# DmSM-1/C-OFDM

Hardware: AMD Instinct MI355X
Metric: IQ-samples/sec (tx IFFT+CP and rx FFT+equalise), 2048-subcarrier frames, 1/2/4/8 GPU (higher is better)
Workload: dtype f64

## Files before the change

### c-ofdm_amd/csrc/ofdm_capi.cpp

```cpp
#include <dlfcn.h>
#include <hip/hip_runtime.h>

#include <algorithm>
#include <climits>
#include <cmath>
#include <complex>
#include <cstdarg>
#include <cstdio>
#include <cstdlib>
#include <chrono>
#include <mutex>
#include <cstring>
#include <iterator>
#include <stdexcept>
#include <string>
#include <vector>

#include "../../include/ofdm_mi355x.h"

#if __has_include(<rccl/rccl.h>)
#include <rccl/rccl.h>
static constexpr int kRcclInt64 = ncclInt64, kRcclSum = ncclSum;
#else
static constexpr int kRcclInt64 = 4, kRcclSum = 0;
// ... 185 lines not shown
    return OFDM_OK;
}

int ofdm_host_alloc(ofdm_ctx* c, size_t bytes, void** h)
{
    if (!c || !h) return fail(OFDM_ERR_INVALID, "null argument");
    HIP_TRY(hipSetDevice(c->device));
    HIP_TRY(hipHostMalloc(h, std::max<size_t>(bytes, 1), hipHostMallocDefault));
    return OFDM_OK;
}
int ofdm_host_free(ofdm_ctx* c, void* h)
{
    if (!c) return fail(OFDM_ERR_INVALID, "null ctx");
    if (h) HIP_TRY(hipHostFree(h));
    return OFDM_OK;
}
int ofdm_stream_create(ofdm_ctx* c, void** st)
{
    if (!c || !st) return fail(OFDM_ERR_INVALID, "null argument");
    HIP_TRY(hipSetDevice(c->device));
    hipStream_t s = nullptr;
    HIP_TRY(hipStreamCreateWithFlags(&s, hipStreamNonBlocking));
    *st = s;
    return OFDM_OK;
}
int ofdm_stream_destroy(ofdm_ctx* c, void* st)
{
    if (!c) return fail(OFDM_ERR_INVALID, "null ctx");
    if (st) {
        HIP_TRY(hipStreamSynchronize((hipStream_t)st));
        rx_queue_release(c, (hipStream_t)st);
        if (c->call_valid && c->call_stream == (hipStream_t)st) c->call_valid = false;
        HIP_TRY(hipStreamDestroy((hipStream_t)st));
    }
    return OFDM_OK;
}
int ofdm_memcpy_d2d(ofdm_ctx* c, void* dst, const void* src, size_t n, void* st)
{
    if (!c) return fail(OFDM_ERR_INVALID, "null ctx");
    if (n) HIP_TRY(hipMemcpyAsync(dst, src, n, hipMemcpyDeviceToDevice, (hipStream_t)st));
    return OFDM_OK;
}
int ofdm_copy(ofdm_ctx* c, void* dst, const void* src, size_t n, void* st)
{
    if (!c) return fail(OFDM_ERR_INVALID, "null ctx");
    if (n && (!dst || !src)) return fail(OFDM_ERR_INVALID, "null argument");
    hipError_t e = ofdm::launch_copy(dst, src, n, (hipStream_t)st);
    if (e != hipSuccess) return hip_fail(e, "copy launch");
    return OFDM_OK;
}
int ofdm_event_create(ofdm_ctx* c, void** ev)
{
    if (!c || !ev) return fail(OFDM_ERR_INVALID, "null argument");
    HIP_TRY(hipSetDevice(c->device));
    hipEvent_t e = nullptr;
    HIP_TRY(hipEventCreateWithFlags(&e, hipEventDisableTiming));
    *ev = e;
    return OFDM_OK;
}
int ofdm_event_record(ofdm_ctx* c, void* ev, void* st)
{
    if (!c || !ev) return fail(OFDM_ERR_INVALID, "null argument");
    HIP_TRY(hipEventRecord((hipEvent_t)ev, (hipStream_t)st));
    return OFDM_OK;
}
int ofdm_event_synchronize(ofdm_ctx* c, void* ev)
{
    if (!c || !ev) return fail(OFDM_ERR_INVALID, "null argument");
    HIP_TRY(hipEventSynchronize((hipEvent_t)ev));
    return OFDM_OK;
}
int ofdm_event_destroy(ofdm_ctx* c, void* ev)
{
    if (!c) return fail(OFDM_ERR_INVALID, "null ctx");
    if (ev) HIP_TRY(hipEventDestroy((hipEvent_t)ev));
    return OFDM_OK;
}

static void fill_tx(const ofdm_ctx* c, ofdm::TxArgs& a, const uint8_t* bytes, size_t nframes, double* iq,
                    size_t stride, int16_t* iq16, const ofdm_channel* ch)
{
    a.tab = c->tables(false);
    a.tx_dead = c->tx_sparse ? c->d_tx_dead : nullptr;
    a.bytes = bytes;
    a.iq = reinterpret_cast<double2*>(iq);
    a.iq16 = iq16;
    a.nframes = (long)nframes;
    a.frame_stride = (long)stride;
    a.S = c->S;
    a.D = c->D;
    a.P = c->P;
    a.cp = c->cp;
    a.k = c->k;
    a.bytes_per_frame = c->geo.bytes_per_frame;
    a.pilot_ampl = (double)c->p.pilot_ampl / 1000;
    a.inv_sqrt_n = 1.0 / std::sqrt((double)c->N);
    a.mult = (double)c->p.mult;
    if (ch && ch->noise_std > 0.0) {
        a.noise_scale = ch->noise_std * M_SQRT1_2;
        a.seed = ch->seed;
        a.sample_offset = ch->sample_offset;
    }
}

int ofdm_tx_modulate(ofdm_ctx* c, const uint8_t* bytes, size_t nframes, double* iq_out, size_t frame_stride,
                     int16_t* iq16_out, const ofdm_channel* ch, void* stream)
{
    if (!c || !bytes || !iq_out) return fail(OFDM_ERR_INVALID, "null argument");
    if (frame_stride < (size_t)c->geo.message_len) return fail(OFDM_ERR_INVALID, "frame_stride < message_len");
    if (!aligned16(iq_out)) return fail(OFDM_ERR_INVALID, "iq_out must be 16-byte aligned");
    if (nframes == 0) return OFDM_OK;
    if (nframes * (size_t)c->S > 0x7fffffffu) return fail(OFDM_ERR_INVALID, "too many symbols in one call");
    ofdm::TxArgs a{};
    fill_tx(c, a, bytes, nframes, iq_out, frame_stride, iq16_out, ch);
    hipError_t e = ofdm::launch_tx(c->logn, a, (hipStream_t)stream);
    if (e != hipSuccess) return hip_fail(e, "tx_kernel launch");
    return OFDM_OK;
}

int ofdm_tx_frames(ofdm_ctx* c, const uint8_t* bytes, size_t nframes, double* frames_out, int16_t* frames16_out,
                   void* stream)
{
    if (!c || !bytes || !frames_out) return fail(OFDM_ERR_INVALID, "null argument");
    if (!aligned16(frames_out)) return fail(OFDM_ERR_INVALID, "frames_out must be 16-byte aligned");
    if (nframes == 0) return OFDM_OK;
    ofdm::TxArgs a{};
    fill_tx(c, a, bytes, nframes, frames_out, (size_t)c->geo.frame_len, frames16_out, nullptr);
    a.header = c->d_header;
    a.header_len = (int)(c->t2 + c->geo.preamble_len);
    a.msg_offset = a.header_len;
    hipError_t e = ofdm::launch_tx(c->logn, a, (hipStream_t)stream);
    if (e != hipSuccess) return hip_fail(e, "tx_kernel launch");
    return OFDM_OK;
}

}

static int rx_demod_impl(ofdm_ctx* c, const double* iq, const int16_t* iq16, size_t nframes, size_t frame_stride,
                         const double* chan, size_t chan_stride, double* constell_out, uint8_t* bytes_out,
                         const uint8_t* ref_bytes, unsigned long long* bit_errors, void* stream,
                         double* read_out = nullptr, const ofdm::SoftArgs* soft = nullptr)
{
    if (!c || (!iq && !iq16)) return fail(OFDM_ERR_INVALID, "null argument");
    if (iq16 && ((uintptr_t)iq16 & 3)) return fail(OFDM_ERR_INVALID, "iq16 must be 4-byte aligned");
    if (frame_stride < (size_t)c->geo.message_len) return fail(OFDM_ERR_INVALID, "frame_stride < message_len");
    if ((iq && !aligned16(iq)) || (chan && !aligned16(chan)) || (constell_out && !aligned16(constell_out)))
        return fail(OFDM_ERR_INVALID, "complex buffers must be 16-byte aligned");
    if ((ref_bytes == nullptr) != (bit_errors == nullptr))
        return fail(OFDM_ERR_INVALID, "ref_bytes and bit_errors go together");
    if (nframes == 0) return OFDM_OK;
    if (nframes > 0x7fffffffu) return fail(OFDM_ERR_INVALID, "too many frames in one call");
    ofdm::RxArgs a{};
    a.tab = c->tables(false);
    a.iq = iq16 ? nullptr : reinterpret_cast<const double2*>(iq);
    a.iq16 = reinterpret_cast<const short2*>(iq16);
    a.nframes = (long)nframes;
    a.frame_stride = (long)frame_stride;
    a.chan = reinterpret_cast<const double2*>(chan);
    a.chan_stride = (long)chan_stride;
    a.constell = reinterpret_cast<double2*>(constell_out);
    a.read_out = reinterpret_cast<double2*>(read_out);
    a.bytes = bytes_out;
    a.ref = ref_bytes;
    a.bit_errors = bit_errors;
    a.S = c->S;
    a.D = c->D;
// ... 1025 lines not shown
```

### c-ofdm_amd/csrc/ofdm_create.cpp

```cpp
#include <hip/hip_runtime.h>

#include <algorithm>
#include <cctype>
#include <climits>
#include <cmath>
#include <fstream>
#include <memory>
#include <string>
#include <unordered_map>
#include <vector>

#include "ofdm_ctx.hpp"
#include "ofdm_sync.hpp"
#include "ofdm_tables.hpp"

namespace tables = ofdm::tables;
using ofdm::DevBuf;
using ofdm::fail;
using ofdm::hip_fail;
using ofdm::twiddles;
using tables::ilog2_exact;

namespace {

// ... 21 lines not shown
            return fail(OFDM_ERR_PARSE, "stol failed for key '%s': %s", key.c_str(), e.what());
        }
    }
    return OFDM_OK;
}

template <class T>
int upload(DevBuf<T>& dst, const std::vector<T>& v)
{
    HIP_TRY(hipMalloc((void**)dst.put(), std::max<size_t>(1, v.size()) * sizeof(T)));
    if (!v.empty()) HIP_TRY(hipMemcpy(dst, v.data(), v.size() * sizeof(T), hipMemcpyHostToDevice));
    return OFDM_OK;
}

std::vector<double2> as_double2(const std::vector<cd>& v)
{
    std::vector<double2> o(v.size());
    for (size_t i = 0; i < v.size(); ++i) o[i] = make_double2(v[i].real(), v[i].imag());
    return o;
}

int validate(const ofdm_params* p)
{
    const long N = p->fft_size, D = p->num_data_subc, P = p->num_pilot_subc, k = p->mod_type;
    if (ilog2_exact(N) < 6 || ilog2_exact(N) > 12)
        return fail(OFDM_ERR_UNSUPPORTED, "fft_size=%ld: the HIP FFT covers powers of two 64..4096", N);
    if (P < 1 || D < P || D % P)
        return fail(OFDM_ERR_UNSUPPORTED, "num_data_subc=%ld must be a positive multiple of num_pilot_subc=%ld", D,
                    P);
    if (P > 256) return fail(OFDM_ERR_UNSUPPORTED, "num_pilot_subc > 256");
    if (!(k == 1 || k == 2 || k == 4 || k == 6 || k == 8))
        return fail(OFDM_ERR_INVALID, "modType=%ld is not one of 1,2,4,6,8 (OFDM/modulation.hpp:11-17)", k);
    if (p->cp_size < 0 || p->cp_size > N) return fail(OFDM_ERR_INVALID, "cp_size out of range");
    if (p->num_symb < 1 || p->num_pr_symb < 1) return fail(OFDM_ERR_INVALID, "num_symb/num_pr_symb must be >= 1");
    if ((D * p->num_symb * k) % 8 || (D * k) % 8)
        return fail(OFDM_ERR_UNSUPPORTED, "num_data_subc*modType must be a multiple of 8 bits");
    if ((D * p->num_pr_symb) % 8) return fail(OFDM_ERR_UNSUPPORTED, "preamble bits must fill bytes");
    tables::Layout lay;
    if (const char* why = tables::carrier_layout(N, D, P, lay)) return fail(OFDM_ERR_INVALID, "%s", why);
    if (p->t2sin_size < 0 || (p->t2sin_size && (p->t2_sin_f1 < 0 || p->t2_sin_f1 >= p->t2sin_size ||
                                                p->t2_sin_f2 < 0 || p->t2_sin_f2 >= p->t2sin_size)))
        return fail(OFDM_ERR_INVALID, "T2 tones outside T2sin_size");
    if (p->pr_sin_len < 0 || p->pr_sin_len > (N + p->cp_size) * p->num_pr_symb)
        return fail(OFDM_ERR_INVALID, "pr_sin_len exceeds the preamble");
    return OFDM_OK;
}


void set_geometry(ofdm_ctx* c, const ofdm_params& p)
{
    c->p = p;
    c->N = (int)p.fft_size;
    c->logn = ilog2_exact(c->N);
    c->D = (int)p.num_data_subc;
    c->P = (int)p.num_pilot_subc;
    c->cp = (int)p.cp_size;
    c->S = (int)p.num_symb;
    c->k = (int)p.mod_type;
    c->L = c->N + c->cp;
    c->seg = c->D / c->P;
    c->npr = (int)p.num_pr_symb;
    c->t2 = (int)p.t2sin_size;
    c->geo = tables::geometry(p);
    ofdm_walk_tuning_default(&c->walk);
    c->ring = std::max(0L, p.rx_buf_size) * c->geo.frame_len;
}

int layout_tables(ofdm_ctx* c)
{
    tables::Layout lay;
    if (const char* why = tables::carrier_layout(c->N, c->D, c->P, lay)) return fail(OFDM_ERR_INVALID, "%s", why);
    for (int j = 0; j < c->P; ++j) {
        c->geo.pilot_bin[j] = lay.pilot[j];
        c->geo.segment_bin[j] = lay.segst[j];
    }
    c->tx_code = tables::tx_code(lay);
    c->tx_dead = ofdm::tx_dead_masks(c->tx_code);
    int rc;
    if (std::any_of(c->tx_dead.begin(), c->tx_dead.end(), [](unsigned m) { return m != 0; }) &&
        (rc = upload(c->d_tx_dead, c->tx_dead)))
        return rc;
    if ((rc = upload(c->d_rx_pack, tables::rx_pack(lay, c->N))) ||
        (rc = upload(c->d_pilot_swz, tables::pilot_swz(lay, c->N))) || (rc = upload(c->d_tx_code, c->tx_code)) ||
        (rc = upload(c->d_tw, twiddles(c->N))) || (rc = upload(c->d_data_bin, lay.data_bin)) ||
        (rc = upload(c->d_data_slot, lay.data_slot)) || (rc = upload(c->d_pilot_bin, lay.pilot)) ||
        (rc = upload(c->d_bin_map, lay.bin_map)) || (rc = upload(c->d_const, tables::constellation(c->k))) ||
        (rc = upload(c->d_const_bpsk, tables::constellation(1))))
        return rc;
    return OFDM_OK;
}

int decision_thresholds(ofdm_ctx* c)
{
    if (c->k != 2) return OFDM_OK;
    DevBuf<double> d_tau;
    double h_tau[4] = {};
    hipError_t e = hipMalloc((void**)d_tau.put(), sizeof(h_tau));
    if (e == hipSuccess) e = ofdm::launch_decide_tau_scan(c->k, d_tau, nullptr);
    if (e == hipSuccess) e = hipMemcpy(h_tau, d_tau, sizeof(h_tau), hipMemcpyDeviceToHost);
    if (e != hipSuccess) return hip_fail(e, "decision threshold scan");
    for (int j = 0; j < 3; ++j) c->dec_tau[j] = h_tau[j];
    c->dec_fast = h_tau[3] == 1.0;
    return OFDM_OK;
}

int synthesize_preamble(ofdm_ctx* c)
{
    const long nb = (long)c->D * c->npr / 8, plen = c->geo.preamble_len;
    c->preamble_bytes = tables::preamble_bytes(nb, c->p.pr_seed);
    DevBuf<uint8_t> d_b;
    DevBuf<double2> d_pre;
    HIP_TRY(hipMalloc((void**)d_b.put(), std::max<long>(1, nb)));
    HIP_TRY(hipMalloc((void**)d_pre.put(), plen * sizeof(double2)));
    HIP_TRY(hipMemcpy(d_b, c->preamble_bytes.data(), nb, hipMemcpyHostToDevice));
    ofdm::TxArgs a{};
    a.tab = c->tables(true);
    a.bytes = d_b;
    a.iq = d_pre;
    a.nframes = 1;
    a.frame_stride = plen;
    a.S = c->npr;
    a.D = c->D;
    a.P = c->P;
    a.cp = c->cp;
    a.k = 1;
    a.bytes_per_frame = nb;
    a.pilot_ampl = (double)c->p.pilot_ampl / 1000;
    a.inv_sqrt_n = 1.0 / std::sqrt((double)c->N);
    a.mult = (double)c->p.mult;
    hipError_t e = ofdm::launch_tx(c->logn, a, nullptr);
    if (e == hipSuccess) e = hipDeviceSynchronize();
    std::vector<double2> pre(plen);
    if (e == hipSuccess) e = hipMemcpy(pre.data(), d_pre, plen * sizeof(double2), hipMemcpyDeviceToHost);
    if (e != hipSuccess) return hip_fail(e, "preamble synthesis");
    c->ofdm_preamble.resize(plen);
    for (long i = 0; i < plen; ++i) c->ofdm_preamble[i] = cd(pre[i].x, pre[i].y);
    return OFDM_OK;
}

int preamble_tables(ofdm_ctx* c)
{
    const ofdm_params& p = c->p;
    c->t2_symbol = tables::t2_symbol(c->t2, p.t2_sin_f1, p.t2_sin_f2);
    c->t2_mask = tables::t2_mask(c->t2, (int)p.t2_sin_f1, (int)p.t2_sin_f2, (int)p.smooth);
    c->mod_preamble = tables::mod_preamble(c->preamble_bytes, (long)c->D * c->npr);
    c->templ = tables::preamble_template(c->ofdm_preamble, (int)p.pr_sin_len);
    std::vector<double2> hdr = as_double2(c->t2_symbol);
    const std::vector<double2> pre = as_double2(c->ofdm_preamble);
    hdr.insert(hdr.end(), pre.begin(), pre.end());
    std::vector<double2> tsp, twm;
    if (p.pr_sin_len <= ofdm::WALK_FFT_M - 63) {
        tsp = tables::template_spectrum(c->templ, ofdm::WALK_FFT_M, &c->tspec_max);
        twm = twiddles(ofdm::WALK_FFT_M);
    }
    std::vector<float2> tsp32(tsp.size());
    for (size_t k = 0; k < tsp.size(); ++k) tsp32[k] = make_float2((float)tsp[k].x, (float)tsp[k].y);
    int rc;
    if ((!tsp.empty() &&
         ((rc = upload(c->d_tspec, tsp)) || (rc = upload(c->d_tspec32, tsp32)) || (rc = upload(c->d_twm, twm)))) ||
        (rc = upload(c->d_header, hdr)) || (rc = upload(c->d_preamble, pre)) ||
        (rc = upload(c->d_templ, as_double2(c->templ))) || (rc = upload(c->d_modpre, as_double2(c->mod_preamble))) ||
        (rc = upload(c->d_t2mask, c->t2_mask)))
        return rc;
    return OFDM_OK;
}

int detector_scratch(ofdm_ctx* c)
{
    int rc;
    if ((rc = upload(c->d_first, std::vector<int>{INT_MAX, 0, 0, 0}))) return rc;
    const size_t cyc = 2 * (size_t)c->p.t2sin_size + (size_t)c->p.pr_sin_len;
    if ((rc = upload(c->d_pre_hv, std::vector<double>(ofdm_ctx::PRE_SCRATCH_STARTS * cyc, 0.0))) ||
        (rc = upload(c->d_pre_done, std::vector<unsigned>(ofdm_ctx::PRE_SCRATCH_STARTS, 0u))))
        return rc;
    if (c->t2 >= 64 && c->t2 <= 4096 && ilog2_exact(c->t2) > 0) {
        c->t2_logn = ilog2_exact(c->t2);
        if ((rc = upload(c->d_t2tw, twiddles(c->t2)))) return rc;
    }
    return OFDM_OK;
}

int rx_counters(ofdm_ctx* c)
{
    const size_t qbytes = ofdm_ctx::RX_QUEUE_SLOTS * 16 * sizeof(int);
    hipError_t qe = hipMalloc((void**)c->d_rxq.put(), qbytes);
    if (qe == hipSuccess) qe = hipMemset(c->d_rxq, 0, qbytes);
    if (qe == hipSuccess) qe = hipDeviceSynchronize();
    if (qe != hipSuccess) return hip_fail(qe, "rx frame counters");
    return OFDM_OK;
}

}

int ofdm::cfo_plan(ofdm_ctx* c, int nsym, ofdm_ctx::CfoPlan** out, hipStream_t st)
{
    for (auto& pl : c->cfo_plans)
        if (pl.nsym == nsym) {
            *out = &pl;
            return OFDM_OK;
// ... 117 lines not shown
```

### c-ofdm_amd/csrc/ofdm_ctx.hpp

```cpp
#pragma once
#include <hip/hip_runtime.h>

#include <complex>
#include <cstddef>
#include <cstdint>
#include <vector>

#include "../../include/ofdm_mi355x.h"
#include "ofdm_internal.hpp"
#include "ofdm_owned.hpp"

using cd = std::complex<double>;

struct ofdm_ctx {
    template <class T>
    using DevBuf = ofdm::DevBuf<T>;
    ofdm_params p{};
    int device = 0;
    int logn = 0;
    int N = 0, D = 0, P = 0, cp = 0, S = 0, k = 0, L = 0, seg = 0, npr = 0, t2 = 0;
    ofdm_geometry geo{};
    std::vector<cd> t2_symbol, ofdm_preamble, mod_preamble, templ;
    std::vector<uint8_t> preamble_bytes;
    std::vector<double> t2_mask;
    DevBuf<double2> d_tw;
    DevBuf<int> d_data_bin;
    DevBuf<int> d_data_slot;
    DevBuf<int> d_pilot_bin;
    DevBuf<int> d_bin_map;
    DevBuf<int> d_rx_pack;
    DevBuf<int> d_pilot_swz;
    DevBuf<int> d_tx_code;
    std::vector<int> tx_code;
    std::vector<unsigned> tx_dead;
    DevBuf<unsigned> d_tx_dead;
#ifndef OFDM_TX_SPARSE_DEFAULT
#define OFDM_TX_SPARSE_DEFAULT 1
#endif
    bool tx_sparse = OFDM_TX_SPARSE_DEFAULT != 0;
    DevBuf<double2> d_const;
    DevBuf<double2> d_const_bpsk;
    double dec_tau[3] = {};
    bool dec_fast = false;
    DevBuf<double2> d_header;
    DevBuf<double2> d_preamble;
    DevBuf<double2> d_templ;
    DevBuf<double2> d_tspec;
    DevBuf<float2> d_tspec32;
    DevBuf<double2> d_twm;
    double tspec_max = 0.0;
    DevBuf<double2> d_modpre;
    DevBuf<double> d_t2mask;
    DevBuf<double2> d_t2tw;
    DevBuf<int> d_first;
    int t2_logn = -1;
    struct CfoPlan {
        int nsym = 0, logm = -1, g = 0;
        DevBuf<double2> tw_sub;
        DevBuf<double2> tw_full;
        DevBuf<int> borders;
    };
    std::vector<CfoPlan> cfo_plans;
    template <class Own>
    struct Grown {
        Own p;
        size_t bytes = 0;
    };
    using Grow = Grown<DevBuf<void>>;
    using GrowHost = Grown<ofdm::HostBlock>;
    Grow d_cfo_scratch, d_scratch;
    Grow s_walk, s_batch, s_chan, s_pbs;
    static constexpr size_t PRE_SCRATCH_STARTS = 64;
    DevBuf<double> d_pre_hv;
    DevBuf<unsigned> d_pre_done;
    GrowHost h_walk, h_frames;
    hipStream_t h_frames_stream = nullptr;
    bool h_frames_used = false;
    DevBuf<int> d_queue;
    static constexpr int RX_QUEUE_SLOTS = 32;
    DevBuf<int> d_rxq;
    hipStream_t rxq_stream[RX_QUEUE_SLOTS] = {};
    bool rxq_live[RX_QUEUE_SLOTS] = {};
    int rxq_used = 0;
    ofdm_walk_tuning walk{};
    long ring = 0;
    bool queue_zero = false;
    ofdm::Event ev_call;
    hipStream_t call_stream = nullptr;
    bool call_valid = false;
    ofdm::Event ev_walk;
    ofdm::Event ev_wdone;
    ofdm::Stream side;
    Grow s_pub, s_chain;
    GrowHost h_status;
    bool pub_zero = false;
    bool phase_timing = false;
    bool phase_valid = false;
    ofdm::Event ev_phase[4];

    ofdm::DevTables tables(bool bpsk) const
    {
        ofdm::DevTables t;
        t.tw = d_tw;
        t.data_bin = d_data_bin;
        t.data_slot = d_data_slot;
        t.pilot_bin = d_pilot_bin;
        t.bin_map = d_bin_map;
        t.rx_pack = d_rx_pack;
        t.pilot_swz = d_pilot_swz;
        t.tx_code = d_tx_code;
        t.constell = bpsk ? d_const_bpsk : d_const;
        return t;
    }
};

// ... 43 lines not shown
```

### c-ofdm_amd/csrc/ofdm_internal.hpp

```cpp
#pragma once
#include <hip/hip_runtime.h>
#include <cmath>
#include <cstdint>
#include <vector>

namespace ofdm {

inline std::vector<double2> twiddles(int n)
{
    std::vector<double2> w(n);
    for (int j = 0; j < n; ++j) {
        const double a = 2.0 * M_PI * (double)j / (double)n;
        w[j] = make_double2(std::cos(a), -std::sin(a));
    }
    return w;
}

struct DevTables {
    const double2* tw;
    const int* data_bin;
    const int* data_slot;
    const int* pilot_bin;
    const int* bin_map;
    const int* rx_pack;
    const int* pilot_swz;
    const int* tx_code;
    const double2* constell;
};

struct TxArgs {
    DevTables tab;
    const uint8_t* bytes;
    const double2* points;
    double2* iq;
    int16_t* iq16;
    const double2* header;
    long nframes;
    long frame_stride;
    long msg_offset;
    int header_len;
    int S, D, P, cp, k;
    long bytes_per_frame;
    double pilot_ampl;
    double inv_sqrt_n;
    double mult;
    double noise_scale;
    unsigned long long seed;
    unsigned long long sample_offset;
    const unsigned* tx_dead;
};

constexpr int CORR_BITS = 9;
constexpr int CORR_PER_SYM = CORR_BITS + 2;

struct RxArgs {
    DevTables tab;
    const double2* iq;
    const short2* iq16;
    long nframes;
    long frame_stride;
    const double2* chan;
    long chan_stride;
    bool chan_recip;
    double2* constell;
    double2* read_out;
    uint8_t* bytes;
    const uint8_t* ref;
    unsigned long long* bit_errors;
    double2* ystage;
    const long* starts;
    long start_off;
    const long* count;
    int* queue;
    const double2* corr;
    int S, D, P, seg, cp, k;
    long bytes_per_frame;
    double pilot_ampl;
    double dec_tau[3];
    int dec_fast;
};

struct SoftArgs {
    void* llr;
    const double* frame_scale;
    double scale;
    int fmt;
};

hipError_t launch_rx_soft(int logn, const RxArgs& a, const SoftArgs& sa, hipStream_t stream);
hipError_t launch_soft_demap(const double2* pts, long n, int k, double scale, int fmt, void* out, hipStream_t stream);
hipError_t launch_tx(int logn, const TxArgs& a, hipStream_t stream);
hipError_t launch_rx(int logn, const RxArgs& a, hipStream_t stream, bool* staged_needed);
hipError_t launch_decide_tau_scan(int k, double* out, hipStream_t stream);
hipError_t launch_copy(void* dst, const void* src, size_t n, hipStream_t stream);
hipError_t launch_demap(double2* pts, long n, int k, uint8_t* bytes, hipStream_t stream);
hipError_t launch_map(const uint8_t* bytes, long nbytes, int k, const double2* table, double2* out,
                      hipStream_t stream);
hipError_t launch_bit_convert(const uint8_t* in, long len, int in_bits, int out_bits, uint8_t* out, long out_len,
                              hipStream_t stream);
hipError_t launch_i16_to_f64(const int16_t* in, long n, double* out, hipStream_t stream);
hipError_t launch_f64_to_i16(const double* in, long n, double mult, int16_t* out, hipStream_t stream);

constexpr int RX_SMAX = 8;
inline int lds_swz_host(int e) { return e ^ ((e >> 3) & 7); }
constexpr int RX_DPT = 4;
constexpr int RX_WAVES_PER_CU = 8;
constexpr int TX_LDS_PILOT = 256, TX_LDS_ZERO = 257;
inline int tx_code_data(int d) { return d | (0xff << 13); }
inline int tx_code_fixed(int entry) { return entry << 21; }
inline std::vector<unsigned> tx_dead_masks(const std::vector<int>& tx_code)
{
    const int T = (int)tx_code.size() / 8;
    std::vector<unsigned> m(T / 64, 0u);
    for (int w = 0; w < T / 64; ++w)
        for (int i = 0; i < 8; ++i) {
            bool dead = true;
            for (int lane = 0; lane < 64; ++lane) dead = dead && tx_code[64 * w + lane + T * i] == tx_code_fixed(TX_LDS_ZERO);
            if (dead) m[w] |= 1u << i;
        }
    return m;
}
constexpr long TX_MAX_GRID = 4096;


struct FecRate { int period, kept; unsigned mask; };
__host__ __device__ inline FecRate fec_rate(int rate)
{
    return rate == 0 ? FecRate{1, 1, 0x1u} : rate == 1 ? FecRate{4, 3, 0x7u} : FecRate{6, 4, 0x27u};
}
constexpr int FEC_TAIL = 6;
constexpr long FEC_MAX_INFO_BITS = 1L << 20;
constexpr int FEC_CW_PER_WG = 4;
constexpr long FEC_LDS_STEPS = 1024;
inline long fec_steps_padded(long info_bits) { return (info_bits + FEC_TAIL + 63) & ~63L; }

struct FecEncArgs {
    const uint8_t* info;
    uint8_t* coded;
    long info_stride, coded_stride;
    long ncw, info_bits, coded_bits;
    int rate;
};

struct FecDecArgs {
    const void* llr;
    long llr_stride;
    long ncw, info_bits;
    unsigned long long* ws;
    uint8_t* out;
    const uint8_t* ref;
    unsigned long long* bit_errors;
    long info_stride;
    int fmt, rate;
    int gather;
};

hipError_t launch_fec_encode(const FecEncArgs& a, hipStream_t stream);
hipError_t launch_fec_decode(const FecDecArgs& a, hipStream_t stream);


constexpr long IL_MAX_BLOCK = 32768;
enum { IL_BITS = 0, IL_I8 = 1, IL_F32 = 2 };

struct IlArgs {
    const void* in;
    void* out;
    long nblocks;
    int n, c, s;
    int kind;
    int dir;
};

struct ScrArgs {
    const uint8_t* in;
    uint8_t* out;
    const uint8_t* seeds;
    long in_stride, out_stride;
    long ncw, nbits;
    unsigned seed;
};

hipError_t launch_interleave(const IlArgs& a, hipStream_t stream);
hipError_t launch_scramble(const ScrArgs& a, hipStream_t stream);

}
```

### c-ofdm_amd/csrc/ofdm_kernels.hip

```cpp
#include <hip/hip_runtime.h>
#include <algorithm>
#include <cstdint>
#include <cstdlib>

#include "ofdm_dev.hpp"
#include "ofdm_fft.hpp"
#include "ofdm_internal.hpp"
#include "ofdm_rx2.hpp"

#include <type_traits>

namespace ofdm {


__device__ __forceinline__ int symbol_bits(const uint8_t* __restrict__ b, long nbytes, long g, int k)
{
    const long bit = g * k;
    const long byte = bit >> 3;
    const int off = (int)(bit & 7);
    const int mask = (1 << k) - 1;
    if (off + k <= 8) return (b[byte] >> (8 - off - k)) & mask;
    const int w = ((int)b[byte] << 8) | (byte + 1 < nbytes ? (int)b[byte + 1] : 0);
    return (w >> (16 - off - k)) & mask;
}

__device__ __forceinline__ int decide(double2 z, int k, double s1, int m)
{
    if (k == 1) return (z.x + z.y) > 0.0;
    const double re = __builtin_fmin(__builtin_fmax(z.x, -1.0), 1.0);
    const double im = __builtin_fmin(__builtin_fmax(z.y, -1.0), 1.0);
    const int ire = (uint8_t)(int)add_rn(mul_rn(add_rn(re, 1.0), s1), 0.5);
    const int iim = (uint8_t)(int)add_rn(mul_rn(add_rn(im, 1.0), s1), 0.5);
    return (ire | (iim * m)) & 0xff;
}

__device__ __forceinline__ double2 clamp_point(double2 z)
{
    return make_double2(z.x < -1.0 ? -1.0 : (1.0 < z.x ? 1.0 : z.x),
                        z.y < -1.0 ? -1.0 : (1.0 < z.y ? 1.0 : z.y));
}

__device__ __forceinline__ uint32_t lowbias32(uint32_t x)
{
    x ^= x >> 16;
    x *= 0x7feb352du;
    x ^= x >> 15;
    x *= 0x846ca68bu;
    x ^= x >> 16;
    return x;
}

struct AwgnKey {
    uint32_t k0, k1;
};

__device__ __forceinline__ AwgnKey awgn_key(unsigned long long seed)
{
    const uint32_t k0 = lowbias32((uint32_t)seed ^ 0x9E3779B9u);
    return {k0, lowbias32((uint32_t)(seed >> 32) + k0)};
}

struct AwgnRun {
    uint32_t lo0, ka, kb;
};

__device__ __forceinline__ AwgnRun awgn_run(AwgnKey key, unsigned long long g0)
{
    const uint32_t hi = (uint32_t)(g0 >> 32);
    return {(uint32_t)g0, lowbias32(hi ^ key.k1) ^ key.k0, lowbias32((hi + 1u) ^ key.k1) ^ key.k0};
}

__device__ __forceinline__ double2 awgn_sample(const AwgnRun& run, uint32_t j, double sc)
{
    const uint32_t lo = run.lo0 + j;
    const uint32_t h1 = lowbias32(lo ^ (lo < run.lo0 ? run.kb : run.ka));
    const uint32_t h2 = h1 * 0x9E3779B9u;
    const float u1 = (float)((h1 >> 8) + 1) * 0x1.0p-24f;
    const float u2 = (float)(h2 >> 8) * 0x1.0p-24f;
    const float r = __builtin_amdgcn_sqrtf(-1.3862943611198906f * __builtin_amdgcn_logf(u1));
    const float c = __builtin_amdgcn_cosf(u2), s = __builtin_amdgcn_sinf(u2);
    return make_double2((double)(r * c) * sc, (double)(r * s) * sc);
}

__device__ __forceinline__ double2 awgn_sample_scaled(const AwgnRun& run, uint32_t j, float scf)
{
    const uint32_t lo = run.lo0 + j;
    const uint32_t h1 = lowbias32(lo ^ (lo < run.lo0 ? run.kb : run.ka));
    const uint32_t h2 = h1 * 0x9E3779B9u;
    const float u1 = (float)((h1 >> 8) + 1) * 0x1.0p-24f;
    const float u2 = (float)(h2 >> 8) * 0x1.0p-24f;
    const float r = __builtin_amdgcn_sqrtf(-1.3862943611198906f * __builtin_amdgcn_logf(u1)) * scf;
    const float c = __builtin_amdgcn_cosf(u2), s = __builtin_amdgcn_sinf(u2);
    return make_double2((double)(r * c), (double)(r * s));
}

__device__ __forceinline__ int16_t to_int16(double v) { return (int16_t)(int)v; }

__device__ __forceinline__ double2 load_untracked(const double2* p)
{
    double2 v;
    asm volatile("global_load_dwordx4 %0, %1, off\n\ts_waitcnt vmcnt(0)" : "=v"(v) : "v"(p) : "memory");
    return v;
}

template <int NT>
__device__ __forceinline__ double block_sum(double v, double* red)
{
#pragma unroll
    for (int o = (NT >= 64 ? 32 : NT / 2); o > 0; o >>= 1) v += __shfl_xor(v, o);
    constexpr int NW = (NT + 63) / 64;
    if constexpr (NW == 1) {
        return v;
    } else {
        const int lane = threadIdx.x & 63, w = threadIdx.x >> 6;
        __syncthreads();
        if (lane == 0) red[w] = v;
        __syncthreads();
        double s = 0.0;
#pragma unroll
        for (int i = 0; i < NW; ++i) s += red[i];
        return s;
    }
}

template <int NT>
__device__ __forceinline__ double block_sum_lds(double v, double* red)
{
#pragma unroll
    for (int o = (NT >= 64 ? 32 : NT / 2); o > 0; o >>= 1) v += __shfl_xor(v, o);
    constexpr int NW = (NT + 63) / 64;
    if constexpr (NW == 1) {
        return v;
    } else {
        const int lane = threadIdx.x & 63, w = threadIdx.x >> 6;
        if (lane == 0) red[w] = v;
        lds_barrier();
        double s = 0.0;
#pragma unroll
        for (int i = 0; i < NW; ++i) s += red[i];
        lds_barrier();
        return s;
    }
}

template <int NT>
__device__ __forceinline__ unsigned long long block_sum_u64(unsigned long long v, double* red)
{
    for (int o = (NT >= 64 ? 32 : NT / 2); o > 0; o >>= 1) v += __shfl_xor(v, o);
    constexpr int NW = (NT + 63) / 64;
    if constexpr (NW == 1) {
        return v;
    } else {
        unsigned long long* r = reinterpret_cast<unsigned long long*>(red);
        const int lane = threadIdx.x & 63, w = threadIdx.x >> 6;
        __syncthreads();
        if (lane == 0) r[w] = v;
        __syncthreads();
        unsigned long long s = 0;
        for (int i = 0; i < NW; ++i) s += r[i];
        return s;
    }
}

constexpr int tx_min_blocks(int logn, bool i16) { return logn == 11 && !i16 ? 4 : 1; }

template <int LOGN, bool POINTS, bool NOISE, bool I16>
__global__ void __launch_bounds__((1 << LOGN) / 8, tx_min_blocks(LOGN, I16)) tx_kernel(TxArgs a)
{
    using FS = FftShape<LOGN>;
    constexpr int N = FS::N, T = FS::T;
    extern __shared__ double2 smem[];
    double2* fft = smem;
    double2* lds_tw = smem + FS::PADN;
    double2* lds_const = lds_tw + TwLds<LOGN>::SIZE;
    uint8_t* sbytes = reinterpret_cast<uint8_t*>(lds_const + TX_LDS_ZERO + 1);
    const int t = threadIdx.x;
    load_twiddles<LOGN>(a.tab.tw, lds_tw, t, T);
    for (int i = t; i < (1 << a.k); i += T) lds_const[i] = a.tab.constell[i];
    if (t == 0) {
        lds_const[TX_LDS_PILOT] = make_double2(a.pilot_ampl, 0.0);
        lds_const[TX_LDS_ZERO] = make_double2(0.0, 0.0);
    }


    const long nsym = a.nframes * a.S;
    const int k = a.k;
    const int bps = a.D * k / 8;
    const int L = N + a.cp;
    auto sym_bytes = [&](long f, int s) { return a.bytes + f * a.bytes_per_frame + (long)s * bps; };
    const bool by_word = (bps & 3) == 0 && (a.bytes_per_frame & 3) == 0 && ((uintptr_t)a.bytes & 3) == 0;
    const int nwords = bps >> 2;
    uint32_t nb[8];
    auto fetch = [&](const uint8_t* src) {
        if (by_word) {
            int tt;
            asm volatile("v_mov_b32 %0, %1" : "=v"(tt) : "v"(t));
            const int wi0 = tt < nwords ? tt : 0, wi1 = tt + T < nwords ? tt + T : 0;
            const uint32_t* w = reinterpret_cast<const uint32_t*>(src);
            nb[0] = w[wi0];
            nb[1] = w[wi1];
        } else {
#pragma unroll
            for (int r = 0; r < 8; ++r) nb[r] = src[t + T * r < bps ? t + T * r : 0];
        }
    };
    auto publish = [&]() {
        if (by_word) {
            uint32_t* w = reinterpret_cast<uint32_t*>(sbytes);
            w[t] = nb[0];
            w[t + T] = nb[1];
        } else {
#pragma unroll
            for (int r = 0; r < 8; ++r) sbytes[t + T * r] = (uint8_t)nb[r];
        }
    };

    long sym = blockIdx.x;
    const long gstep_f = gridDim.x / a.S;
    const int gstep_s = (int)(gridDim.x - gstep_f * a.S);
    long f = sym / a.S;
    int s = (int)(sym - f * a.S);
    if (!POINTS && sym < nsym) {
        fetch(sym_bytes(f, s));
        publish();
    }
    lds_barrier();

    const bool cp_reg = (a.cp % T) == 0;
    const int i_cp = 8 - a.cp / T;
    const int kmask = (1 << k) - 1;

    unsigned dead = 0;
    if constexpr (T >= 64) {
        if (a.tx_dead) dead = __builtin_amdgcn_readfirstlane(a.tx_dead[t >> 6]);
    }

    for (; sym < nsym; sym += gridDim.x) {
        long fn = f + gstep_f;
        int sn = s + gstep_s;
        if (sn >= a.S) {
            sn -= a.S;
            ++fn;
        }
        const bool more = sym + gridDim.x < nsym;
        double2 v[8];
        auto map_first = [&](auto zeros) {
            constexpr int ZEROS = decltype(zeros)::value;
            int code[8];
            {
                int tt;
                asm volatile("v_mov_b32 %0, %1" : "=v"(tt) : "v"(t));
                const int* ct = a.tab.tx_code + tt;
#pragma unroll
                for (int i = 0; i < 8; ++i)
                    if (!((ZEROS >> i) & 1)) code[i] = ct[T * i];
            }
#pragma unroll
            for (int i = 0; i < 8; ++i) {
                if ((ZEROS >> i) & 1) {
                    v[i] = make_double2(0.0, 0.0);
                    continue;
                }
                const int d = code[i] & 0x1fff, m = (code[i] >> 13) & 0xff, base = code[i] >> 21;
                if constexpr (POINTS) {
                    v[i] = m ? a.points[sym * a.D + d] : lds_const[base];
                } else {
                    const int bit = (int)__umul24((unsigned)d, (unsigned)k);
                    const int byte = bit >> 3, off = bit & 7;
                    const int w = ((int)sbytes[byte] << 8) | (int)sbytes[byte + 1];
                    v[i] = lds_const[((w >> (16 - off - k)) & kmask & m) + base];
                }
            }
            if constexpr (!POINTS) fetch(more ? sym_bytes(fn, sn) : sym_bytes(f, s));
            if constexpr (ZEROS == DFT8_FULL)
                stockham_pass<LOGN, 8, 1, +1>(v, t, lds_tw, fft);
            else
                fft_regs_first<LOGN, +1, ZEROS>(v, t, fft);
        };
        if constexpr (T >= 64) {
            if ((dead & DFT8_Z2345) == DFT8_Z2345)
                map_first(std::integral_constant<int, DFT8_Z2345>());
            else if ((dead & DFT8_Z34) == DFT8_Z34)
                map_first(std::integral_constant<int, DFT8_Z34>());
            else
                map_first(std::integral_constant<int, DFT8_FULL>());
        } else {
            map_first(std::integral_constant<int, DFT8_FULL>());
        }
        fft_regs_tail<LOGN, 1, +1>(v, t, lds_tw, fft);
        if constexpr (!POINTS) publish();

        const long base = f * a.frame_stride + a.msg_offset + (long)s * L;
        double2* out = a.iq + base;
        int16_t* out16 = I16 ? a.iq16 + 2 * base : nullptr;
        const unsigned long long g0 = a.sample_offset + (unsigned long long)sym * L;
        const AwgnRun run = NOISE ? awgn_run(awgn_key(a.seed), g0) : AwgnRun{};
        auto emit = [&](int j, double2 z) {
            if constexpr (NOISE && !I16) {
                const double2 w = awgn_sample_scaled(run, (uint32_t)j, (float)a.noise_scale);
                store_nt(out + j, make_double2(fma(z.x, a.inv_sqrt_n, w.x), fma(z.y, a.inv_sqrt_n, w.y)));
                return;
            }
            z.x *= a.inv_sqrt_n;
            z.y *= a.inv_sqrt_n;
            if constexpr (I16) {
                const uint32_t w = (uint16_t)to_int16(z.x * a.mult) | ((uint32_t)(uint16_t)to_int16(z.y * a.mult) << 16);
                __builtin_nontemporal_store(w, reinterpret_cast<uint32_t*>(out16 + 2 * j));
            }
            if constexpr (NOISE) {
                const double2 w = awgn_sample(run, (uint32_t)j, a.noise_scale);
                z.x += w.x;
                z.y += w.y;
            }
            store_nt(out + j, z);
        };
        if (cp_reg) {
#pragma unroll
            for (int i = 0; i < 8; ++i)
                if (i >= i_cp) emit(t + T * i - (N - a.cp), v[i]);
        } else {
            int tt;
            asm volatile("v_mov_b32 %0, %1" : "=v"(tt) : "v"(t));
            lds_barrier();
#pragma unroll
            for (int i = 0; i < 8; ++i)
                if (tt + T * i >= N - a.cp) fft[lds_swz(tt + T * i)] = v[i];
            lds_barrier();
            for (int j = tt; j < a.cp; j += T) emit(j, fft[lds_swz(N - a.cp + j)]);
        }
#pragma unroll
        for (int i = 0; i < 8; ++i) emit(a.cp + t + T * i, v[i]);
        if (a.header && s == 0) {
            double2* fr = a.iq + f * a.frame_stride;
            int16_t* fr16 = I16 ? a.iq16 + 2 * f * a.frame_stride : nullptr;
            for (int j = t; j < a.header_len; j += T) {
                const double2 z = a.header[j];
                fr[j] = z;
                if constexpr (I16) {
                    fr16[2 * j] = to_int16(z.x * a.mult);
                    fr16[2 * j + 1] = to_int16(z.y * a.mult);
                }
            }
        }
        lds_barrier();
        f = fn;
        s = sn;
    }
}

template <int LOGN, bool I16>
struct SymbolRegs;

template <int LOGN>
struct SymbolRegs<LOGN, false> {
    double2 r[8];
    __device__ __forceinline__ void load(const RxArgs& a, long off, int t)
    {
        constexpr int T = (1 << LOGN) / 8;
#pragma unroll
        for (int i = 0; i < 8; ++i)
            r[i] = load_nt(a.iq + off + t + T * i);
    }
    __device__ __forceinline__ double2 get(int i) const { return r[i]; }
};

template <int LOGN>
struct SymbolRegs<LOGN, true> {
    int r[8];
    __device__ __forceinline__ void load(const RxArgs& a, long off, int t)
    {
        constexpr int T = (1 << LOGN) / 8;
        const int* p = reinterpret_cast<const int*>(a.iq16 + off);
#pragma unroll
        for (int i = 0; i < 8; ++i) r[i] = __builtin_nontemporal_load(p + t + T * i);
    }
    __device__ __forceinline__ double2 get(int i) const
    {
        return make_double2((double)(int)(short)(r[i] & 0xffff), (double)(r[i] >> 16));
    }
};

template <int LOGN, bool I16>
__device__ __forceinline__ void dma_symbol(const RxArgs& a, long off, void* stage, int t)
{
    constexpr int T = (1 << LOGN) / 8;
    constexpr int ESZ = I16 ? 4 : 16;
    const int w0 = t & ~63;
#pragma unroll
    for (int i = 0; i < 8; ++i) {
        const int e0 = w0 + T * i;
        const char* g = I16 ? reinterpret_cast<const char*>(a.iq16 + off + e0 + (t & 63))
                            : reinterpret_cast<const char*>(a.iq + off + e0 + (t & 63));
        const unsigned lds = __builtin_amdgcn_readfirstlane(
            (unsigned)(uintptr_t)(__attribute__((address_space(3))) char*)((char*)stage + (size_t)e0 * ESZ));
        unsigned keep;
        if constexpr (I16)
            asm volatile(
                "s_mov_b32 %0, m0\n\t"
                "s_mov_b32 m0, %2\n\t"
                "s_nop 0\n\t"
                "global_load_lds_dword %1, off nt\n\t"
                "s_mov_b32 m0, %0"
                : "=&s"(keep)
                : "v"(g), "s"(lds)
                : "memory");
        else
            asm volatile(
                "s_mov_b32 %0, m0\n\t"
                "s_mov_b32 m0, %2\n\t"
                "s_nop 0\n\t"
                "global_load_lds_dwordx4 %1, off nt\n\t"
                "s_mov_b32 m0, %0"
                : "=&s"(keep)
                : "v"(g), "s"(lds)
// ... 604 lines not shown
```

### c-ofdm_amd/csrc/ofdm_tables.hpp

```cpp
#pragma once
#include <algorithm>
#include <cmath>
#include <complex>
#include <cstdint>
#include <random>
#include <vector>

#include "../../include/ofdm_mi355x.h"
#include "ofdm_internal.hpp"

namespace ofdm::tables {

using cd = std::complex<double>;

inline int ilog2_exact(long n)
{
    if (n <= 0 || (n & (n - 1))) return -1;
    int l = 0;
    while ((1L << l) < n) ++l;
    return l;
}

inline ofdm_geometry geometry(const ofdm_params& p)
{
    const int L = (int)p.fft_size + (int)p.cp_size, D = (int)p.num_data_subc, S = (int)p.num_symb;
    const int npr = (int)p.num_pr_symb, t2 = (int)p.t2sin_size, k = (int)p.mod_type;
    ofdm_geometry g{};
    g.symbol_len = L;
    g.message_len = (long)L * S;
    g.preamble_len = (long)L * npr;
    g.frame_len = t2 + g.preamble_len + g.message_len;
    g.ring_len = g.frame_len * (p.rx_buf_size + 1);
    g.data_per_frame = (long)D * S;
    g.bytes_per_frame = (long)D * S * k / 8;
    g.segment_size = D / (int)p.num_pilot_subc;
    return g;
}

struct Layout {
    std::vector<int> pilot, segst, data_bin, data_slot, bin_map;
};

inline const char* carrier_layout(long N, long D, long P, Layout& o)
{
    const long step = D / P + 1, seg = D / P, half = P / 2;
    o = Layout{};
    o.pilot.assign(P, 0);
    o.segst.assign(P, 0);
    o.bin_map.assign(N, -1);
    long j = 0;
    auto take = [&](long b, long what) {
        if (b < 1 || b >= N || o.bin_map[b] != -1) return false;
        o.bin_map[b] = (int)what;
        return true;
    };
    auto slot = [&](long pilot, long first) -> const char* {
        if (!take(pilot, -2)) return "pilot comb does not fit fft_size";
        o.pilot[j] = (int)pilot;
        o.segst[j] = (int)first;
        for (long t = 0; t < seg; ++t) {
            if (!take(first + t, j * seg + t)) return "data segments do not fit fft_size";
            o.data_bin.push_back((int)(first + t));
            o.data_slot.push_back((int)j);
        }
        return nullptr;
    };
    const char* why = nullptr;
    for (long pos = 1 + seg; j < half && !why; ++j, pos += step) why = slot(pos, pos - seg);
    for (long pos = N - step * half; j < P && !why; ++j, pos += step) why = slot(pos, pos + 1);
    return why;
}

inline std::vector<int> rx_pack(const Layout& l, int N)
{
    const int D = (int)l.data_bin.size();
    std::vector<int> t(std::max(D, RX_DPT * (N / 8)), 0);
    for (int d = 0; d < D; ++d) t[d] = lds_swz_host(l.data_bin[d]) | (l.data_slot[d] << 16);
    return t;
}

inline std::vector<int> pilot_swz(const Layout& l, int N)
{
    const int P = (int)l.pilot.size();
    std::vector<int> t(std::max(P, N / 8), 0);
    for (int j = 0; j < P; ++j) t[j] = lds_swz_host(l.pilot[j]);
    return t;
}

inline std::vector<int> tx_code(const Layout& l)
{
    std::vector<int> t(l.bin_map.size());
    for (size_t b = 0; b < t.size(); ++b)
        t[b] = l.bin_map[b] >= 0 ? tx_code_data(l.bin_map[b])
                                 : tx_code_fixed(l.bin_map[b] == -2 ? TX_LDS_PILOT : TX_LDS_ZERO);
    return t;
}

inline std::vector<double2> constellation(int k)
{
    std::vector<double2> t(1u << k);
    if (k == 1) {
        const double step = M_PI * 2 / (double)2;
        for (int i = 0; i < 2; ++i) {
            const cd z = std::exp(cd(0.0, 1.0) * (step * cd(i) + M_PI_4 * 5));
            t[i] = make_double2(z.real(), z.imag());
        }
    } else {
        const unsigned num = 1u << (k / 2);
        for (unsigned i = 0; i < t.size(); ++i) {
            const uint8_t in = (uint8_t)i;
            t[i] = make_double2(2.0 / (num - 1) * double(in % num) - 1.0, 2.0 / (num - 1) * double(in >> (k / 2)) - 1.0);
        }
    }
    return t;
}

inline std::vector<cd> t2_symbol(int t2, long f1, long f2)
{
    std::vector<cd> sym(t2, cd(0, 0));
    if (t2) {
        std::vector<cd> spec(t2, cd(0, 0));
        spec[f1] = cd(0.5, 0);
        spec[f2] = cd(0.5, 0);
        for (int n = 0; n < t2; ++n) {
            cd acc(0, 0);
            for (int kk = 0; kk < t2; ++kk) {
                if (spec[kk] == cd(0, 0)) continue;
                const double a = 2.0 * M_PI * (double)(((long)kk * n) % t2) / (double)t2;
                acc += spec[kk] * cd(std::cos(a), std::sin(a));
            }
            sym[n] = acc;
        }
    }
    return sym;
}

inline std::vector<double> t2_mask(int t2, int f1, int f2, int sm)
{
    std::vector<double> mask(std::max(1, t2), 0.0);
    if (t2) {
        for (int i = std::max(0, f1 - sm); i <= std::min(t2 - 1, f1 + sm); ++i) mask[i] += 1.0;
        for (int i = std::max(0, f2 - sm); i <= std::min(t2 - 1, f2 + sm); ++i) mask[i] += 1.0;
    }
    return mask;
}

inline std::vector<uint8_t> preamble_bytes(long nb, long seed)
{
    std::vector<uint8_t> bytes(nb);
    std::mt19937 rng(seed);
    std::uniform_int_distribution<int> dist(0, 255);
    for (auto& b : bytes) b = (uint8_t)dist(rng);
    return bytes;
}

inline std::vector<cd> mod_preamble(const std::vector<uint8_t>& bytes, long npoints)
{
    const auto bp = constellation(1);
    std::vector<cd> mp(npoints);
    for (long i = 0; i < npoints; ++i) {
        const int bit = (bytes[i >> 3] >> (7 - (i & 7))) & 1;
        mp[i] = cd(bp[bit].x, bp[bit].y);
    }
    return mp;
}

inline std::vector<cd> preamble_template(const std::vector<cd>& ofdm_preamble, int Lt)
{
    std::vector<cd> templ(Lt);
    double norm = 0.0;
    for (int i = 0; i < Lt; ++i) {
        templ[i] = std::conj(ofdm_preamble[i]);
        norm += std::abs(templ[i] * templ[i]);
    }
    norm = std::sqrt(norm);
    for (int i = 0; i < Lt; ++i) templ[i] /= cd(norm);
    return templ;
}

inline std::vector<double2> template_spectrum(const std::vector<cd>& templ, int M, double* max_abs)
// ... 48 lines not shown
```

Baseline: 148.6 billion.

## Precompute per-bin tx bit-extraction descriptors and hoist AWGN wrap check per symbol

Adds a host-built per-bin descriptor table (shift, byte index, constellation entry) so the tx mapper extracts bits with a single ubfe and one-byte loads for k in {1,2,4,8}, replacing the per-bin multiply, mask and two-byte assembly. It also specialises the emit path on whether the AWGN counter wraps within the symbol, removing the per-sample key select, and rewrites output addressing as base plus thread offset. A self-test checks that the descriptors match the old formula. The cost is an extra device table and more template variants.

```diff
diff --git a/c-ofdm_amd/apps/txmap_selftest.cpp b/c-ofdm_amd/apps/txmap_selftest.cpp
--- /dev/null
+++ b/c-ofdm_amd/apps/txmap_selftest.cpp
@@ -0,0 +1,70 @@
+#include <cstdio>
+#include <cstdlib>
+#include <vector>
+
+#include "../csrc/ofdm_tables.hpp"
+
+namespace T = ofdm::tables;
+
+static int g_bad = 0;
+
+static void check(bool ok, const char* what, int k, int bin)
+{
+    if (ok || g_bad++) return;
+    fprintf(stderr, "txmap_selftest: %s (k = %d, bin %d)\n", what, k, bin);
+}
+
+int main(int argc, char** argv)
+{
+    if (argc != 4) {
+        fprintf(stderr, "txmap_selftest: need fft_size, num_data_subc, num_pilot_subc\n");
+        return 2;
+    }
+    const long N = atol(argv[1]), D = atol(argv[2]), P = atol(argv[3]);
+    if (T::ilog2_exact(N) < 6 || T::ilog2_exact(N) > 12 || P < 1 || P > 256 || D < P || D % P) {
+        fprintf(stderr, "txmap_selftest: geometry outside what ofdm_create accepts\n");
+        return 2;
+    }
+    T::Layout lay;
+    if (const char* why = T::carrier_layout(N, D, P, lay)) {
+        printf("%s\n", why);
+        return 1;
+    }
+    const std::vector<int> code = T::tx_code(lay);
+    for (int k = 1; k <= 8; ++k) {
+        const std::vector<int> map = T::tx_map(lay, k);
+        const bool one = ofdm::tx_map_one_byte(k);
+        const int kmask = (1 << k) - 1;
+        long pairs = 0;
+        check((long)map.size() == N, "table size", k, -1);
+        for (int b = 0; b < (int)N && !g_bad; ++b) {
+            const int d = code[b] & 0x1fff, m = (code[b] >> 13) & 0xff, base = code[b] >> 21;
+            const int bit = d * k, byte = bit >> 3, off = bit & 7;
+            const unsigned sh = ofdm::tx_map_shift(map[b]), mb = ofdm::tx_map_byte(map[b]),
+                           ent = ofdm::tx_map_entry(map[b]);
+            check(map[b] >= 0, "descriptor is negative", k, b);
+            check(sh <= (one ? 8u : 16u), "shift out of range", k, b);
+            check(ent <= (unsigned)ofdm::TX_LDS_ZERO, "table entry out of range", k, b);
+            check(mb + (one ? 0u : 1u) < (unsigned)N, "byte index outside the kernel's N-byte stage", k, b);
+            check(m ? (int)mb == byte : mb == 0, "byte index", k, b);
+            if (!m) check(sh == (one ? 8u : 16u), "a fixed bin's shift must leave 0", k, b);
+            auto same = [&](unsigned b0, unsigned b1) {
+                const int w = (int)((b0 << 8) | b1);
+                const int want = ((w >> (16 - off - k)) & kmask & m) + base;
+                const unsigned wd = one ? b0 : (unsigned)w;
+                const unsigned got = ((wd >> sh) & (unsigned)kmask) + ent;
+                ++pairs;
+                return got == (unsigned)want;
+            };
+            bool ok = true;
+            for (unsigned x = 0; x < 256; ++x)
+                ok = ok && same(x, 0x00) && same(x, 0xff) && same(0x00, x) && same(0xff, x) &&
+                     same(x, (x * 167u + 13u) & 0xff);
+            check(ok, "descriptor and formula differ", k, b);
+        }
+        if (g_bad) return 1;
+        printf("k=%d %s form: %ld bins, %ld byte pairs equal\n", k, one ? "one-byte" : "two-byte", N, pairs);
+    }
+    printf("txmap_selftest: ok\n");
+    return 0;
+}
diff --git a/c-ofdm_amd/csrc/ofdm_capi.cpp b/c-ofdm_amd/csrc/ofdm_capi.cpp
--- a/c-ofdm_amd/csrc/ofdm_capi.cpp
+++ b/c-ofdm_amd/csrc/ofdm_capi.cpp
@@ -291,6 +291,7 @@
 {
     a.tab = c->tables(false);
     a.tx_dead = c->tx_sparse ? c->d_tx_dead : nullptr;
+    a.tx_map = c->d_tx_map;
     a.bytes = bytes;
     a.iq = reinterpret_cast<double2*>(iq);
     a.iq16 = iq16;
diff --git a/c-ofdm_amd/csrc/ofdm_create.cpp b/c-ofdm_amd/csrc/ofdm_create.cpp
--- a/c-ofdm_amd/csrc/ofdm_create.cpp
+++ b/c-ofdm_amd/csrc/ofdm_create.cpp
@@ -127,7 +127,8 @@
         return rc;
     if ((rc = upload(c->d_rx_pack, tables::rx_pack(lay, c->N))) ||
         (rc = upload(c->d_pilot_swz, tables::pilot_swz(lay, c->N))) || (rc = upload(c->d_tx_code, c->tx_code)) ||
-        (rc = upload(c->d_tw, twiddles(c->N))) || (rc = upload(c->d_data_bin, lay.data_bin)) ||
+        (rc = upload(c->d_tx_map, tables::tx_map(lay, c->k))) ||
+        (rc = upload(c->d_tx_map_bpsk, tables::tx_map(lay, 1))) || (rc = upload(c->d_tw, twiddles(c->N))) || (rc = upload(c->d_data_bin, lay.data_bin)) ||
         (rc = upload(c->d_data_slot, lay.data_slot)) || (rc = upload(c->d_pilot_bin, lay.pilot)) ||
         (rc = upload(c->d_bin_map, lay.bin_map)) || (rc = upload(c->d_const, tables::constellation(c->k))) ||
         (rc = upload(c->d_const_bpsk, tables::constellation(1))))
@@ -160,6 +161,7 @@
     HIP_TRY(hipMemcpy(d_b, c->preamble_bytes.data(), nb, hipMemcpyHostToDevice));
     ofdm::TxArgs a{};
     a.tab = c->tables(true);
+    a.tx_map = c->d_tx_map_bpsk;
     a.bytes = d_b;
     a.iq = d_pre;
     a.nframes = 1;
diff --git a/c-ofdm_amd/csrc/ofdm_ctx.hpp b/c-ofdm_amd/csrc/ofdm_ctx.hpp
--- a/c-ofdm_amd/csrc/ofdm_ctx.hpp
+++ b/c-ofdm_amd/csrc/ofdm_ctx.hpp
@@ -31,6 +31,8 @@
     DevBuf<int> d_rx_pack;
     DevBuf<int> d_pilot_swz;
     DevBuf<int> d_tx_code;
+    DevBuf<int> d_tx_map;
+    DevBuf<int> d_tx_map_bpsk;
     std::vector<int> tx_code;
     std::vector<unsigned> tx_dead;
     DevBuf<unsigned> d_tx_dead;
diff --git a/c-ofdm_amd/csrc/ofdm_internal.hpp b/c-ofdm_amd/csrc/ofdm_internal.hpp
--- a/c-ofdm_amd/csrc/ofdm_internal.hpp
+++ b/c-ofdm_amd/csrc/ofdm_internal.hpp
@@ -48,6 +48,7 @@
     unsigned long long seed;
     unsigned long long sample_offset;
     const unsigned* tx_dead;
+    const int* tx_map;
 };
 
 constexpr int CORR_BITS = 9;
@@ -120,6 +121,17 @@
         }
     return m;
 }
+__host__ __device__ inline bool tx_map_one_byte(int k) { return k == 1 || k == 2 || k == 4 || k == 8; }
+inline int tx_map_word(int shift, int byte, int entry) { return shift | (byte << 5) | (entry << 21); }
+inline int tx_map_data(int d, int k)
+{
+    const int bit = d * k, off = bit & 7;
+    return tx_map_word((tx_map_one_byte(k) ? 8 : 16) - off - k, bit >> 3, 0);
+}
+inline int tx_map_fixed(int entry, int k) { return tx_map_word(tx_map_one_byte(k) ? 8 : 16, 0, entry); }
+__host__ __device__ inline unsigned tx_map_shift(int w) { return (unsigned)w & 31u; }
+__host__ __device__ inline unsigned tx_map_byte(int w) { return ((unsigned)w >> 5) & 0xfffu; }
+__host__ __device__ inline unsigned tx_map_entry(int w) { return (unsigned)w >> 21; }
 constexpr long TX_MAX_GRID = 4096;
 
 
diff --git a/c-ofdm_amd/csrc/ofdm_kernels.hip b/c-ofdm_amd/csrc/ofdm_kernels.hip
--- a/c-ofdm_amd/csrc/ofdm_kernels.hip
+++ b/c-ofdm_amd/csrc/ofdm_kernels.hip
@@ -70,10 +70,19 @@
     return {(uint32_t)g0, lowbias32(hi ^ key.k1) ^ key.k0, lowbias32((hi + 1u) ^ key.k1) ^ key.k0};
 }
 
+__device__ __forceinline__ bool awgn_run_wraps(const AwgnRun& run, uint32_t n) { return run.lo0 + (n - 1u) < run.lo0; }
+
+template <bool UNIFORM>
+__device__ __forceinline__ uint32_t awgn_hash(const AwgnRun& run, uint32_t j)
+{
+    const uint32_t lo = run.lo0 + j;
+    return lowbias32(lo ^ (UNIFORM || lo >= run.lo0 ? run.ka : run.kb));
+}
+
+template <bool UNIFORM = false>
 __device__ __forceinline__ double2 awgn_sample(const AwgnRun& run, uint32_t j, double sc)
 {
-    const uint32_t lo = run.lo0 + j;
-    const uint32_t h1 = lowbias32(lo ^ (lo < run.lo0 ? run.kb : run.ka));
+    const uint32_t h1 = awgn_hash<UNIFORM>(run, j);
     const uint32_t h2 = h1 * 0x9E3779B9u;
     const float u1 = (float)((h1 >> 8) + 1) * 0x1.0p-24f;
     const float u2 = (float)(h2 >> 8) * 0x1.0p-24f;
@@ -82,10 +91,10 @@
     return make_double2((double)(r * c) * sc, (double)(r * s) * sc);
 }
 
+template <bool UNIFORM = false>
 __device__ __forceinline__ double2 awgn_sample_scaled(const AwgnRun& run, uint32_t j, float scf)
 {
-    const uint32_t lo = run.lo0 + j;
-    const uint32_t h1 = lowbias32(lo ^ (lo < run.lo0 ? run.kb : run.ka));
+    const uint32_t h1 = awgn_hash<UNIFORM>(run, j);
     const uint32_t h2 = h1 * 0x9E3779B9u;
     const float u1 = (float)((h1 >> 8) + 1) * 0x1.0p-24f;
     const float u2 = (float)(h2 >> 8) * 0x1.0p-24f;
@@ -228,7 +237,7 @@
 
     const bool cp_reg = (a.cp % T) == 0;
     const int i_cp = 8 - a.cp / T;
-    const int kmask = (1 << k) - 1;
+    const bool one_byte = tx_map_one_byte(k);
 
     unsigned dead = 0;
     if constexpr (T >= 64) {
@@ -250,26 +259,36 @@
             {
                 int tt;
                 asm volatile("v_mov_b32 %0, %1" : "=v"(tt) : "v"(t));
-                const int* ct = a.tab.tx_code + tt;
+                const int* ct = (POINTS ? a.tab.tx_code : a.tx_map) + tt;
 #pragma unroll
                 for (int i = 0; i < 8; ++i)
                     if (!((ZEROS >> i) & 1)) code[i] = ct[T * i];
             }
-#pragma unroll
-            for (int i = 0; i < 8; ++i) {
-                if ((ZEROS >> i) & 1) {
-                    v[i] = make_double2(0.0, 0.0);
-                    continue;
+            auto map_bytes = [&](auto one) {
+                constexpr bool ONE = decltype(one)::value;
+#pragma unroll
+                for (int i = 0; i < 8; ++i) {
+                    if ((ZEROS >> i) & 1) continue;
+                    const unsigned byte = tx_map_byte(code[i]);
+                    const unsigned w = ONE ? (unsigned)sbytes[byte] : ((unsigned)sbytes[byte] << 8) | sbytes[byte + 1];
+                    const unsigned bits = __builtin_amdgcn_ubfe(w, (unsigned)code[i], (unsigned)k);
+                    v[i] = lds_const[bits + tx_map_entry(code[i])];
                 }
-                const int d = code[i] & 0x1fff, m = (code[i] >> 13) & 0xff, base = code[i] >> 21;
-                if constexpr (POINTS) {
+            };
+#pragma unroll
+            for (int i = 0; i < 8; ++i)
+                if ((ZEROS >> i) & 1) v[i] = make_double2(0.0, 0.0);
+            if constexpr (POINTS) {
+#pragma unroll
+                for (int i = 0; i < 8; ++i) {
+                    if ((ZEROS >> i) & 1) continue;
+                    const int d = code[i] & 0x1fff, m = (code[i] >> 13) & 0xff, base = code[i] >> 21;
                     v[i] = m ? a.points[sym * a.D + d] : lds_const[base];
-                } else {
-                    const int bit = (int)__umul24((unsigned)d, (unsigned)k);
-                    const int byte = bit >> 3, off = bit & 7;
-                    const int w = ((int)sbytes[byte] << 8) | (int)sbytes[byte + 1];
-                    v[i] = lds_const[((w >> (16 - off - k)) & kmask & m) + base];
                 }
+            } else if (one_byte) {
+                map_bytes(std::true_type());
+            } else {
+                map_bytes(std::false_type());
             }
             if constexpr (!POINTS) fetch(more ? sym_bytes(fn, sn) : sym_bytes(f, s));
             if constexpr (ZEROS == DFT8_FULL)
@@ -295,41 +314,58 @@
         int16_t* out16 = I16 ? a.iq16 + 2 * base : nullptr;
         const unsigned long long g0 = a.sample_offset + (unsigned long long)sym * L;
         const AwgnRun run = NOISE ? awgn_run(awgn_key(a.seed), g0) : AwgnRun{};
-        auto emit = [&](int j, double2 z) {
-            if constexpr (NOISE && !I16) {
-                const double2 w = awgn_sample_scaled(run, (uint32_t)j, (float)a.noise_scale);
-                store_nt(out + j, make_double2(fma(z.x, a.inv_sqrt_n, w.x), fma(z.y, a.inv_sqrt_n, w.y)));
-                return;
+        auto emit_symbol = [&](auto uni) {
+            constexpr bool UNI = decltype(uni)::value;
+            auto emit = [&](int ju, int tl, double2 z) {
+                const uint32_t j = (uint32_t)(ju + tl);
+                double2* p = reinterpret_cast<double2*>(reinterpret_cast<char*>(out + ju) + ((uint32_t)tl << 4));
+                if constexpr (NOISE && !I16) {
+                    const double2 w = awgn_sample_scaled<UNI>(run, j, (float)a.noise_scale);
+                    store_nt(p, make_double2(fma(z.x, a.inv_sqrt_n, w.x), fma(z.y, a.inv_sqrt_n, w.y)));
+                    return;
+                }
+                z.x *= a.inv_sqrt_n;
+                z.y *= a.inv_sqrt_n;
+                if constexpr (I16) {
+                    const uint32_t w = (uint16_t)to_int16(z.x * a.mult) | ((uint32_t)(uint16_t)to_int16(z.y * a.mult) << 16);
+                    __builtin_nontemporal_store(
+                        w, reinterpret_cast<uint32_t*>(reinterpret_cast<char*>(out16 + 2 * ju) + ((uint32_t)tl << 2)));
+                }
+                if constexpr (NOISE) {
+                    const double2 w = awgn_sample<UNI>(run, j, a.noise_scale);
+                    z.x += w.x;
+                    z.y += w.y;
+                }
+                store_nt(p, z);
+            };
+            int first = i_cp, cpl = a.cp;
+            asm volatile("" : "+s"(first), "+s"(cpl));
+            if (cp_reg) {
+#pragma unroll
+                for (int i = 0; i < 8; ++i)
+                    if (i >= first) emit(T * (i - first), t, v[i]);
+            } else {
+                int tt;
+                asm volatile("v_mov_b32 %0, %1" : "=v"(tt) : "v"(t));
+                lds_barrier();
+#pragma unroll
+                for (int i = 0; i < 8; ++i)
+                    if (tt + T * i >= N - a.cp) fft[lds_swz(tt + T * i)] = v[i];
+                lds_barrier();
+                for (int ju = 0; ju < a.cp; ju += T)
+                    if (ju + tt < a.cp) emit(ju, tt, fft[lds_swz(N - a.cp + ju + tt)]);
             }
-            z.x *= a.inv_sqrt_n;
-            z.y *= a.inv_sqrt_n;
-            if constexpr (I16) {
-                const uint32_t w = (uint16_t)to_int16(z.x * a.mult) | ((uint32_t)(uint16_t)to_int16(z.y * a.mult) << 16);
-                __builtin_nontemporal_store(w, reinterpret_cast<uint32_t*>(out16 + 2 * j));
-            }
-            if constexpr (NOISE) {
-                const double2 w = awgn_sample(run, (uint32_t)j, a.noise_scale);
-                z.x += w.x;
-                z.y += w.y;
-            }
-            store_nt(out + j, z);
+#pragma unroll
+            for (int i = 0; i < 8; ++i) emit(cpl + T * i, t, v[i]);
         };
-        if (cp_reg) {
-#pragma unroll
-            for (int i = 0; i < 8; ++i)
-                if (i >= i_cp) emit(t + T * i - (N - a.cp), v[i]);
+        if constexpr (NOISE) {
+            if (awgn_run_wraps(run, (uint32_t)L))
+                emit_symbol(std::false_type());
+            else
+                emit_symbol(std::true_type());
         } else {
-            int tt;
-            asm volatile("v_mov_b32 %0, %1" : "=v"(tt) : "v"(t));
-            lds_barrier();
-#pragma unroll
-            for (int i = 0; i < 8; ++i)
-                if (tt + T * i >= N - a.cp) fft[lds_swz(tt + T * i)] = v[i];
-            lds_barrier();
-            for (int j = tt; j < a.cp; j += T) emit(j, fft[lds_swz(N - a.cp + j)]);
-        }
-#pragma unroll
-        for (int i = 0; i < 8; ++i) emit(a.cp + t + T * i, v[i]);
+            emit_symbol(std::false_type());
+        }
         if (a.header && s == 0) {
             double2* fr = a.iq + f * a.frame_stride;
             int16_t* fr16 = I16 ? a.iq16 + 2 * f * a.frame_stride : nullptr;
diff --git a/c-ofdm_amd/csrc/ofdm_tables.hpp b/c-ofdm_amd/csrc/ofdm_tables.hpp
--- a/c-ofdm_amd/csrc/ofdm_tables.hpp
+++ b/c-ofdm_amd/csrc/ofdm_tables.hpp
@@ -96,6 +96,15 @@
     return t;
 }
 
+inline std::vector<int> tx_map(const Layout& l, int k)
+{
+    std::vector<int> t(l.bin_map.size());
+    for (size_t b = 0; b < t.size(); ++b)
+        t[b] = l.bin_map[b] >= 0 ? tx_map_data(l.bin_map[b], k)
+                                 : tx_map_fixed(l.bin_map[b] == -2 ? TX_LDS_PILOT : TX_LDS_ZERO, k);
+    return t;
+}
+
 inline std::vector<double2> constellation(int k)
 {
     std::vector<double2> t(1u << k);
```

Result: no change. 150.1 billion, median of 6 (+1.0%).
